# Project-MONAI/GenerativeModels

Measured on AMD Instinct MI355X. Metric: 3D volumes/sec (DDIM 50-step sample, 1x128^3), higher is better.
Workload: dtype bf16; 1 GPU; C2: 3D DiffusionModelUNet(64,128,256; 2 res blocks; mid-block attention 1 head x 256) DDIM-50 sampling of 1x1x128^3 volumes, 1 volume per GPU per step; inference_steps=50, parallelism=1 independent replicas (batch-sharded, no data-path collective), hip_graph=False, self_launched=False

## Files before the change

### generativemodels_amd/csrc/conv_dma.hip

```cpp
#include "conv_dma_shared.h"
#include <type_traits>

#ifdef GM_CONV_TIMELINE
#define TL_STAMP(k)                                                                                                              \
  do {                                                                                                                           \
    if ((p.debug_flags & 4096) && threadIdx.x == 0 && tl_on)                                                                            \
      reinterpret_cast<unsigned long long*>(p.kpartial)[(long long)blockIdx.x * 64 + (k)] = __builtin_readcyclecounter();        \
  } while (0)
#else
#define TL_STAMP(k)
#endif
#ifndef GM_DMA_PART
#define GM_DMA_PART (-1)
#endif
#define DMA_PART(k) (GM_DMA_PART == -1 || GM_DMA_PART == (k))
static __device__ __attribute__((aligned(64))) unsigned int gm_zero_row[16] = {0};

template <typename T, int NW, int MF, int S, int MINW, int KS = 3, int NFR_ = 4, bool PRE = false>
__global__ __launch_bounds__(64 * NW, MINW) void conv_dma_kernel(const GmConvDesc p, const unsigned phase_wgs, const unsigned phase_sleeps) {
  constexpr int BK = ConvTraits<T>::BK;
  constexpr int VECW = ConvTraits<T>::VECW;
  constexpr int NT = 64 * NW;
  constexpr int NFR = NFR_, G = KS == 3 ? 3 : 2, RING = KS == 3 ? 3 : 4;
  static_assert(KS == 3 || (KS == 2 && S == 1 && (NW == 8 || NW == 4)), "the sub-pixel variant is stride 1, 8 waves x 32 or 4 waves x 64 voxels");
  static_assert(NW * MF * 16 == 512 || NW * MF * 16 == (S == 1 ? 256 : 128), "waves x fragments cover the tile");
  constexpr int TH = 4, TW = 16, BM = NW * MF * 16, TD = BM / (TH * TW);
  constexpr int NPW = KS == 2 ? 2 : 1;
  constexpr int PD = S * (TD - 1) + KS, PH = S * (TH - 1) + KS, PW = S * (TW - 1) + KS + (NPW - 1);
  constexpr int EW = TW + 1;
  constexpr int PLANE = ((PH * PW + 15) / 16) * 16;
  constexpr int PROWS = PD * PLANE;
  constexpr int PPIECES = PROWS / 16;
  constexpr int PPW = (PPIECES + NW - 1) / NW;
  constexpr int BN = 16 * NFR;
  constexpr int WROWS = G * BN;
  constexpr bool WGEN = NFR != 4 || (KS == 2 && NW == 4);
  constexpr int PATCH_BYTES = PROWS * DMA_ROWB;
  constexpr int WBUF_BYTES = WROWS * DMA_ROWB;
  constexpr int PVT_OFF = PATCH_BYTES + (KS == 2 ? 36864 : RING * WBUF_BYTES) + 512;
  constexpr int NGROUPS = KS * KS * KS / G * NPW;
  constexpr int WPW = WGEN ? WROWS / 16 / NW : (KS == 2 ? 1 : (NW == 8 ? 2 : (NW == 4 ? 3 : 1)));
  static_assert(!WGEN || (S == 1 && (WROWS / 16) % NW == 0), "general panel distribution: whole pieces per wave");
  static_assert(WROWS == (KS == 3 ? 3 : 2) * BN, "G taps per weight panel");
  static_assert(NGROUPS % RING == 0, "the ring slot of a group is a compile-time constant");
  constexpr bool DIRECT_W = NFR == 4 && KS == 3;

  extern __shared__ __attribute__((aligned(1024))) char smem[];
  const unsigned lds0 = (unsigned)(uintptr_t)smem;

  const int tid = threadIdx.x;
  const int lane = tid & 63;
  const int wave = __builtin_amdgcn_readfirstlane(tid >> 6);
  const int l15 = lane & 15, q = lane >> 4;
  if (blockIdx.x < phase_wgs) {
    const unsigned tg = __builtin_amdgcn_s_getreg((3 << 11) | (16 << 6) | 4);
    if (tg & 1) {
      for (unsigned k = phase_sleeps; k > 0; --k) __builtin_amdgcn_s_sleep(16);
    }
  }

  const int Dt = KS == 2 ? p.Ds : p.Do, Ht = KS == 2 ? p.Hs : p.Ho, Wt = KS == 2 ? p.Ws : p.Wo;
  const int ntd = (Dt + TD - 1) / TD, nth = (Ht + TH - 1) / TH, ntw = (Wt + TW - 1) / TW;
  const int ncb = (p.Cout + BN - 1) / BN;
  const int ksplit = (KS == 3 && S == 1 && p.kpartial && p.ksplit > 1) ? p.ksplit : 1;
  int Dv = p.Ds, Hv = p.Hs, Wv = p.Ws;
  if (p.in_mode == 1) { Dv *= p.fd; Hv *= p.fh; Wv *= p.fw; }
  const int nchunks = p.Cin / BK;
  const int cout_pad = (p.Cout + 15) & ~15;
  const int cps = ksplit > 1 ? (nchunks + ksplit - 1) / ksplit : nchunks;
// ... 32 lines not shown
  int psw = 0;
#pragma unroll
  for (int j = 0; j < PPW; ++j) {
    const int row = 16 * (wave + NW * j) + (lane >> 2);
    const int rr = row % PLANE;
    psw |= dma_swz(rr % PW) << (2 * j);
  }
  int pvox[PPW];
  constexpr bool PVOX_LDS = KS == 2 && NW == 4;
  int* pvt = reinterpret_cast<int*>(smem + PVT_OFF) + threadIdx.x;
  if (PVOX_LDS) pvt[PPW * NT] = psw;
  auto place_patch = [&](const Tile& t) __attribute__((always_inline)) {
    KDesc& pk = cold_desc();
    const int ud0 = t.td_i * TD * S - (KS == 2 ? 1 - ((t.par >> 1) & 1) : pk.pd), uh0 = t.th_i * TH * S - (KS == 2 ? 1 - (t.par & 1) : pk.ph),
              uw0 = t.tw_i * TW * S - (KS == 2 ? 1 : pk.pw);
    OPAQUE_LANE(lane_p);
#pragma unroll
    for (int j = 0; j < PPW; ++j) {
      const int row = 16 * (wave + NW * j) + (lane_p >> 2);
      const int pa = row / PLANE, rr = row - pa * PLANE;
      const int pb = rr / PW, lc = rr - pb * PW;
      const int pc = S == 1 ? lc : (lc < EW ? 2 * lc : 2 * (lc - EW) + 1);
      int ud = ud0 + pa, uh = uh0 + pb, uw = uw0 + pc;
      const bool ok = (row < PROWS) & (rr < PH * PW) & (ud >= 0) & (ud < Dv) & (uh >= 0) & (uh < Hv) & (uw >= 0) & (uw < Wv);
      if (pk.in_mode == 1) { ud /= pk.fd; uh /= pk.fh; uw /= pk.fw; }
      const int pvj = ok ? ((t.n * pk.Ds + ud) * pk.Hs + uh) * pk.Ws + uw : -1;
      if (PVOX_LDS) pvt[j * NT] = pvj; else pvox[j] = pvj;
    }
  };
  const long long xrowb = p.x_ld * (long long)sizeof(T);
  const char* x2base = reinterpret_cast<const char*>(p.x2);
  const long long x2rowb = p.x2_ld * (long long)sizeof(T);
  const int nchunks0 = p.x2 ? p.cin_split / BK : nchunks;
  auto issue_patch = [&](int chunk) __attribute__((always_inline)) {
#ifdef GM_CONV_ABLATE
    if (p.debug_flags & 1024) return;
#endif
    const bool second = chunk >= nchunks0;
    const char* cbase = second ? x2base + (long long)(chunk - nchunks0) * (BK * (int)sizeof(T)) : xbase + (long long)chunk * (BK * (int)sizeof(T));
    const long long rowb = second ? x2rowb : xrowb;
#pragma unroll
    for (int j = 0; j < PPW; ++j) {
      if (wave + NW * j < PPIECES) {
        int pv = PVOX_LDS ? pvt[j * NT] : pvox[j];
        asm volatile("" : "+v"(pv));
        int ps = PVOX_LDS ? pvt[PPW * NT] : psw;
        if (PVOX_LDS) asm volatile("" : "+v"(ps));
        const char* src = pv >= 0 ? cbase + pv * rowb + (((lane & 3) ^ ((ps >> (2 * j)) & 3)) << 4) : zero + ((lane & 3) << 4);
        dma16(src, lds0 + (unsigned)(16 * (wave + NW * j)) * DMA_ROWB);
      }
    }
  };

  Tile cur = decode(sx + pos);
  const Tile stride = decode(gx);
  place_patch(cur);
  if (min(nchunks, cur.ks * cps) < nchunks) issue_patch(min(nchunks, cur.ks * cps));

  constexpr bool pre = PRE;
  float sc[VECW], sh[VECW];
  auto load_affine = [&](int chunk) __attribute__((always_inline)) {
    const int c0 = chunk * BK + (lane & 3) * VECW;
    const float* ps = p.pre_scale + (long long)cur.n * p.Cin + c0;
    const float* ph = p.pre_shift + (long long)cur.n * p.Cin + c0;
#pragma unroll
    for (int i = 0; i < VECW; i += 4) {
      const float4 a = *reinterpret_cast<const float4*>(ps + i), b = *reinterpret_cast<const float4*>(ph + i);
      sc[i] = a.x; sc[i + 1] = a.y; sc[i + 2] = a.z; sc[i + 3] = a.w;
      sh[i] = b.x; sh[i + 1] = b.y; sh[i + 2] = b.z; sh[i + 3] = b.w;
    }
  };
  auto transform_patch = [&]() __attribute__((always_inline)) {
#pragma unroll
    for (int j = 0; j < PPW; ++j) {
      if (wave + NW * j < PPIECES && pvox[j] >= 0) {
        char* a = smem + (16 * (wave + NW * j) + (lane >> 2)) * DMA_ROWB + (((lane & 3) ^ ((psw >> (2 * j)) & 3)) << 4);
        float v[VECW];
        Vec16<T>::unpack(*reinterpret_cast<const uint4*>(a), v);
#pragma unroll
        for (int i = 0; i < VECW; ++i) v[i] = v[i] * sc[i] + sh[i];
        conv_act_vec(v, p.pre_act, sizeof(T) == 4);
        *reinterpret_cast<uint4*>(a) = Vec16<T>::pack(v);
      }
    }
    asm volatile("s_waitcnt lgkmcnt(0)" ::: "memory");
  };


  const char* wbase = nullptr;
  int wsrc[WPW];
  auto place_weights = [&](const Tile& t) __attribute__((always_inline)) {
    KDesc& pk = cold_desc();
    wbase = reinterpret_cast<const char*>(pk.w) + (long long)(t.par * NPW) * nchunks * (KS * KS * KS) * cout_pad * DMA_ROWB;
    OPAQUE_LANE(lane_w);
#pragma unroll
    for (int h = 0; h < WPW; ++h) {
      const int row = WGEN ? 16 * (wave + NW * h) + (lane_w >> 2)
                    : KS == 2 ? 16 * wave + (lane_w >> 2)
                              : NW == 8 ? (h == 0 ? 16 * wave + (lane_w >> 2) : 128 + 8 * wave + ((lane_w & 31) >> 2))
                                        : (NW == 4 ? 16 * (wave + NW * h) + (lane_w >> 2) : 16 * (wave < 12 ? wave : 0) + (lane_w >> 2));
      const int u = row / BN, col = row % BN;
      const int co = t.cb * BN + (DIRECT_W ? direct_col_chan<T>(col) : col);
      wsrc[h] = co < cout_pad ? ((u * cout_pad + co) * DMA_ROWB + (((lane_w & 3) ^ dma_swz(row)) << 4)) : -1;
    }
  };
  auto issue_w_pieces = [&](int t, int buf, int h0, int h1) __attribute__((always_inline)) {
#ifdef GM_CONV_ABLATE
    if (p.debug_flags & 512) return;
#endif
    const char* panel = KS == 2 ? wbase + ((long long)((t & 7) >> 2) * nchunks * 8 + (long long)(t >> 3) * 8 + 2 * (t & 3)) * cout_pad * DMA_ROWB
                                : wbase + (long long)t * G * cout_pad * DMA_ROWB;
    const unsigned dst = lds0 + PATCH_BYTES + (unsigned)buf * WBUF_BYTES;
#pragma unroll
    for (int h = h0; h < h1; ++h) {
      const char* src = wsrc[h] >= 0 ? panel + wsrc[h] : zero + ((lane & 3) << 4);
      if (WGEN) {
        dma16(src, dst + (unsigned)(16 * (wave + NW * h)) * DMA_ROWB);
      } else if (KS == 2) {
        dma16(src, dst + (unsigned)(16 * wave) * DMA_ROWB);
      } else if (NW == 8) {
        if (h == 0) dma16(src, dst + (unsigned)(16 * wave) * DMA_ROWB);
        else if (lane < 32) dma16(src, dst + (unsigned)(128 + 8 * wave) * DMA_ROWB);
      } else if (NW == 16) {
        if (wave < 12) dma16(src, dst + (unsigned)(16 * wave) * DMA_ROWB);
      } else {
        dma16(src, dst + (unsigned)(16 * (wave + NW * h)) * DMA_ROWB);
      }
    }
  };
  auto issue_w = [&](int t, int buf) __attribute__((always_inline)) { issue_w_pieces(t, buf, 0, WPW); };


  constexpr int SCRATCH_WAVE = MF * 16 * 144, SCRATCH_BYTES = NW * SCRATCH_WAVE;
  constexpr int RING_BYTES = KS == 2 ? (RING * WBUF_BYTES > 36864 ? RING * WBUF_BYTES : 36864) : RING * WBUF_BYTES;
  constexpr bool EARLY = SCRATCH_BYTES <= RING_BYTES;
  constexpr int SCRATCH_OFF = EARLY ? PATCH_BYTES : 0;
  static_assert(EARLY || SCRATCH_BYTES <= PATCH_BYTES + RING_BYTES, "the transpose scratch fits under the addend vector");
  static_assert(BN * 8 <= SCRATCH_WAVE, "a wave's statistic partials fit into its scratch block");
  static_assert(PVT_OFF == PATCH_BYTES + RING_BYTES + 512, "the placement table follows the addend vector");
  float* addv = reinterpret_cast<float*>(smem + PATCH_BYTES + RING_BYTES);
  constexpr bool DIRECT = NFR == 4 && KS == 3;
  constexpr int EPASSES = (NFR * 16 * (int)sizeof(T) + 127) / 128;
  constexpr int CH_PER_PASS = 128 / (int)sizeof(T);
  static_assert(EPASSES <= 4, "at most 4 epilogue passes (128 output channels in fp32)");

  for (;;) {
#ifdef GM_CONV_TIMELINE
    const bool tl_on = pos == tl_pos;
#endif
    TL_STAMP(0);
    const int c_begin = min(nchunks, cur.ks * cps), c_end = min(nchunks, c_begin + cps);
    const int total = (c_end - c_begin) * NGROUPS;
    const int od0 = cur.td_i * TD, oh0 = cur.th_i * TH, ow0 = cur.tw_i * TW;
    TL_STAMP(1);
    place_weights(cur);
    if (total > 0) {
      issue_w(c_begin * NGROUPS, 0);
      if (total > 1) issue_w(c_begin * NGROUPS + 1, 1);
      if (pre) load_affine(c_begin);
    }
    float addend = 0.f;
    KDesc& pa = cold_desc();
    OPAQUE_LANE(lane_a);
    const int tid_a = wave * 64 + lane_a;
    if (tid_a < BN) {
      const int co = cur.cb * BN + tid_a;
      if (co < pa.Cout) {
        if (pa.bias) addend += pa.bias[co];
        if (pa.skip_bias) addend += pa.skip_bias[co];
        if (pa.rowvec) addend += pa.rowvec[(long long)cur.n * pa.rowvec_bstride + co];
      }
    }
    TL_STAMP(55);
    constexpr int HK = S * (MF - 1) + KS;
    static_assert(MF <= 4 && (4 % MF) == 0, "a wave's fragments stay inside one 4-row tile plane");
    OPAQUE_LANE(lane_t);
    const int l15t = lane_t & 15, qt = lane_t >> 4;
    constexpr int NXA = KS + NPW - 1;
    int xa[NXA];
    {
      const int m0 = wave * MF * 16 + l15t;
      const int a = m0 >> 6, bb0 = (m0 >> 4) & 3, c = m0 & 15;
#pragma unroll
      for (int kw = 0; kw < NXA; ++kw) {
        const int col = S == 1 ? c + kw : (kw == 1 ? EW + c : c + (kw >> 1));
        xa[kw] = (S * a * PLANE + S * bb0 * PW + col) * DMA_ROWB + ((qt ^ dma_swz(col)) << 4);
      }
    }
    const int wa0 = PATCH_BYTES + l15t * DMA_ROWB + ((qt ^ dma_swz(l15t)) << 4);
#define XADDR(hk, kw) (xa[kw] + (hk) * (PW * DMA_ROWB))
#define WADDR(nf) (wa0 + (nf) * (16 * DMA_ROWB))
    f32x4_t accs[NPW][NFR][MF];
#pragma unroll
    for (int pw = 0; pw < NPW; ++pw)
#pragma unroll
      for (int nf = 0; nf < NFR; ++nf)
#pragma unroll
        for (int mf = 0; mf < MF; ++mf) accs[pw][nf][mf] = (f32x4_t){0.f, 0.f, 0.f, 0.f};
    f32x4_t (&acc)[NFR][MF] = accs[0];
    if (tid_a < BN) addv[tid_a] = addend;
    TL_STAMP(56);
    if (total > 0) {
      dma_wait<0>();
      if (pre) transform_patch();
    }
    __builtin_amdgcn_s_barrier();
#ifdef GM_CONV_TIMELINE
    if (p.debug_flags & 2048) {
      const unsigned tg = __builtin_amdgcn_s_getreg((3 << 11) | (16 << 6) | 4);
      if (tg & 1) {
        for (int k = (p.debug_flags >> 16) & 255; k > 0; --k) __builtin_amdgcn_s_sleep(1);
      }
    }
#endif
    TL_STAMP(2);

    for (int chunk = c_begin; chunk < c_end; ++chunk) {
      const bool last_chunk = chunk + 1 == c_end;
      constexpr int NH = NFR / 4;
      constexpr bool PIPE2 = NH == 1 && !PRE && (KS == 2 || S == 2 || MINW == 2);
      if constexpr (PIPE2) {
        uint4 xf[2][MF], wf[2][4];
        auto read_tap = [&](int g, int u, int set) __attribute__((always_inline)) {
          const int tap = (KS == 2 ? g % 4 : g) * G + u;
          const int kd = tap / (KS * KS), kh = (tap / KS) % KS, kw = tap % KS + (KS == 2 ? g / 4 : 0);
#pragma unroll
          for (int nf = 0; nf < 4; ++nf)
            wf[set][nf] = *reinterpret_cast<const uint4*>(smem + WADDR(nf) + (g % RING) * WBUF_BYTES + u * (BN * DMA_ROWB));
#pragma unroll
          for (int mf = 0; mf < MF; ++mf)
            xf[set][mf] = *reinterpret_cast<const uint4*>(smem + XADDR(S * mf + kh, kw) + kd * (PLANE * DMA_ROWB));
        };
        auto mma_tap_pw = [&](int set, int pw) __attribute__((always_inline)) {
#pragma unroll
          for (int nf = 0; nf < 4; ++nf)
#pragma unroll
            for (int mf = 0; mf < MF; ++mf) Mma<T>::run(wf[set][nf], xf[set][mf], accs[pw][nf][mf]);
        };
#define mma_tap(set) mma_tap_pw(set, KS == 2 ? g / 4 : 0)
        constexpr int NMMA = MF * 4 * (sizeof(T) == 2 ? 1 : 4), NRD = MF + 4;
        static_assert(G == 3 || G == 2, "taps per panel");
#pragma unroll
        for (int g = 0; g < NGROUPS; ++g) {
          const int t = chunk * NGROUPS + g;
          const int X = (g * G) & 1, Y = X ^ 1;
          const int LASTSET = (g * G + G - 1) & 1, NEXTSET = ((g + 1) * G) & 1;
          if (g == 0) read_tap(0, 0, X);
          read_tap(g, 1, Y);
          mma_tap(X);
          if (g == 0) __builtin_amdgcn_sched_group_barrier(0x100, 2 * NRD, 0);
          else __builtin_amdgcn_sched_group_barrier(0x100, NRD, 0);
          __builtin_amdgcn_sched_group_barrier(0x008, NMMA, 0);
          if (g < NGROUPS - 2 || !last_chunk) issue_w(t + 2, (g + 2) % RING);
          if (G == 3) {
            read_tap(g, 2, X);
            mma_tap(Y);
            __builtin_amdgcn_sched_group_barrier(0x100, NRD, 0);
            __builtin_amdgcn_sched_group_barrier(0x008, NMMA, 0);
          }
          if (g == NGROUPS - 1) {
            if (!last_chunk) {
              asm volatile("s_waitcnt lgkmcnt(0)" ::: "memory");
              __builtin_amdgcn_s_barrier();
              issue_patch(chunk + 1);
              if (pre) load_affine(chunk + 1);
              dma_wait<0>();
              if (pre) transform_patch();
              __builtin_amdgcn_s_barrier();
            }
          } else {
            if ((g < NGROUPS - 2 || !last_chunk) && (NW != 16 || wave < 12)) dma_wait<WPW>(); else dma_wait<0>();
            __builtin_amdgcn_s_barrier();
            read_tap(g + 1, 0, NEXTSET);
          }
          mma_tap(LASTSET);
          if (g < NGROUPS - 1) {
            __builtin_amdgcn_sched_group_barrier(0x100, NRD, 0);
            __builtin_amdgcn_sched_group_barrier(0x008, NMMA, 0);
          }
          if (chunk - c_begin < 5) TL_STAMP(3 + (chunk - c_begin) * 10 + g);
        }
      } else {
#pragma unroll
      for (int g = 0; g < NGROUPS; ++g) {
        const int t = chunk * NGROUPS + g;
        if (g < NGROUPS - 2 || !last_chunk) issue_w(t + 2, (g + 2) % RING);
        constexpr int NSTEPS = G * NH;
        uint4 xf[MF], wf[4];
        auto read_step = [&](int st) __attribute__((always_inline)) {
          const int u = st / NH, hf = st % NH;
          const int tap = g * G + u;
          const int kd = tap / (KS * KS), kh = (tap / KS) % KS, kw = tap % KS;
#pragma unroll
          for (int nf = 0; nf < 4; ++nf)
            wf[nf] = *reinterpret_cast<const uint4*>(smem + WADDR(nf) + hf * (64 * DMA_ROWB) + (g % RING) * WBUF_BYTES + u * (BN * DMA_ROWB));
          if (hf == 0) {
#pragma unroll
            for (int mf = 0; mf < MF; ++mf)
              xf[mf] = *reinterpret_cast<const uint4*>(smem + XADDR(S * mf + kh, kw) + kd * (PLANE * DMA_ROWB));
          }
        };
        auto mma_step = [&](int st) __attribute__((always_inline)) {
          const int hf = st % NH;
#pragma unroll
          for (int nf = 0; nf < 4; ++nf)
#pragma unroll
            for (int mf = 0; mf < MF; ++mf) Mma<T>::run(wf[nf], xf[mf], acc[hf * 4 + nf][mf]);
        };
        constexpr int NMMA = MF * 4 * (sizeof(T) == 2 ? 1 : 4);
#pragma unroll
        for (int st = 0; st < NSTEPS - 1; ++st) {
          read_step(st);
          mma_step(st);
          if (st % NH == 0) __builtin_amdgcn_sched_group_barrier(0x100, MF + 4, 0);
// ... 110 lines not shown
              dma16(src, lds0 + (unsigned)(j * BM + wave * (MF * 16) + h * 16) * DMA_ROWB);
            }
            if (WGEN || NW == 4 || (wave >> 2) == j) {
              const char* src = wco < cout_pad ? wsk + ((long long)sc * cout_pad + wco) * DMA_ROWB + wswz : zero + ((lane_k & 3) << 4);
              dma16(src, lds0 + PATCH_BYTES + (unsigned)(j * BN + wpiece * 16) * DMA_ROWB);
            }
          }
        }
        asm volatile("s_waitcnt vmcnt(0)" ::: "memory");
        __builtin_amdgcn_s_barrier();
  #pragma unroll
        for (int j = 0; j < 2; ++j) {
          if (sc0 + j < nsc) {
            uint4 xf[MF], wf[4];
  #pragma unroll
            for (int mf = 0; mf < MF; ++mf) xf[mf] = *reinterpret_cast<const uint4*>(smem + caddr[mf] + j * (BM * DMA_ROWB));
  #pragma unroll
            for (int hf = 0; hf < NFR / 4; ++hf) {
  #pragma unroll
              for (int nf = 0; nf < 4; ++nf)
                wf[nf] = *reinterpret_cast<const uint4*>(smem + WADDR(nf) + hf * (64 * DMA_ROWB) + j * (BN * DMA_ROWB));
  #pragma unroll
              for (int nf = 0; nf < 4; ++nf)
  #pragma unroll
                for (int mf = 0; mf < MF; ++mf) Mma<T>::run(wf[nf], xf[mf], acc[hf * 4 + nf][mf]);
            }
          }
        }
      }
    }


    TL_STAMP(61);
    const bool has_next = pos + gx < cx;
    const bool has_next_early = !DIRECT || has_next || partial;
    if (has_next_early) {
      asm volatile("s_waitcnt lgkmcnt(0)" ::: "memory");
      __builtin_amdgcn_s_barrier();
    }
    Tile nxt = cur;
    if (has_next) {
      if (ksplit > 1) {
        nxt = decode(sx + pos + gx);
      } else {
        int c;
        nxt.cb = cur.cb + stride.cb; c = nxt.cb >= ncb ? 1 : 0; nxt.cb -= c ? ncb : 0;
        if (KS == 2) { nxt.par = cur.par + stride.par + c; c = nxt.par >> 2; nxt.par &= 3; }
        nxt.tw_i = cur.tw_i + stride.tw_i + c; c = nxt.tw_i >= ntw ? 1 : 0; nxt.tw_i -= c ? ntw : 0;
        nxt.th_i = cur.th_i + stride.th_i + c; c = nxt.th_i >= nth ? 1 : 0; nxt.th_i -= c ? nth : 0;
        nxt.td_i = cur.td_i + stride.td_i + c; c = nxt.td_i >= ntd ? 1 : 0; nxt.td_i -= c ? ntd : 0;
        nxt.n = cur.n + stride.n + c;
      }
      place_patch(nxt);
      if (EARLY && min(nchunks, nxt.ks * cps) < nchunks) issue_patch(min(nchunks, nxt.ks * cps));
    }
    TL_STAMP(57);
    KDesc& pe = cold_desc();
    if (KS == 3 && S == 1 && ksplit > 1) {
      const long long nv = (long long)pe.N * pe.Do * pe.Ho * pe.Wo;
      float* part = pe.kpartial + (long long)cur.ks * nv * pe.Cout;
  #pragma unroll
      for (int mf = 0; mf < MF; ++mf) {
        const int m = (wave * MF + mf) * 16 + (lane_e & 15);
        const int od = od0 + (m >> 6), oh = oh0 + ((m >> 4) & 3), ow = ow0 + (m & 15);
        if (od < pe.Do && oh < pe.Ho && ow < pe.Wo) {
          float* row = part + ((((long long)cur.n * pe.Do + od) * pe.Ho + oh) * pe.Wo + ow) * pe.Cout;
  #pragma unroll
          for (int nf = 0; nf < NFR; ++nf) {
            const int co = cur.cb * BN + (DIRECT ? direct_chan<T>(nf, lane_e >> 4, 0) : nf * 16 + (lane_e >> 4) * 4);
            if (co < pe.Cout)
              *reinterpret_cast<float4*>(row + co) = make_float4(acc[nf][mf][0], acc[nf][mf][1], acc[nf][mf][2], acc[nf][mf][3]);
          }
        }
      }
    } else {

#ifdef GM_CONV_ABLATE
    if (!(pe.debug_flags & 256)) {
#endif
    if (DIRECT && d_direct) {
      const int qe = lane_e >> 4;
      typedef float f32x2_t __attribute__((ext_vector_type(2)));
      f32x2_t ds[NST][VECW / 2], dq[NST][VECW / 2];
#pragma unroll
      for (int st = 0; st < NST; ++st)
#pragma unroll
        for (int i = 0; i < VECW / 2; ++i) { ds[st][i] = (f32x2_t){0.f, 0.f}; dq[st][i] = (f32x2_t){0.f, 0.f}; }
      const int Dl = KS == 2 ? pe.Ds : pe.Do, Hl = KS == 2 ? pe.Hs : pe.Ho, Wl = KS == 2 ? pe.Ws : pe.Wo;
      const bool has_res = pe.res != nullptr, has_stats = pe.stats != nullptr;
      const bool full = od0 + TD <= Dl && oh0 + TH <= Hl && ow0 + TW <= Wl && (cur.cb + 1) * BN <= pe.Cout;
      bool ok_st[NST];
#pragma unroll
      for (int st = 0; st < NST; ++st) ok_st[st] = d_lane_ok && cur.cb * BN + (64 * st + 16 * qe) / (int)sizeof(T) < pe.Cout;
      f32x2_t addl[NST][VECW / 2];
#pragma unroll
      for (int st = 0; st < NST; ++st)
#pragma unroll
        for (int i = 0; i < VECW; i += 4) {
          const float4 a = *reinterpret_cast<const float4*>(addv + (64 * st) / (int)sizeof(T) + qe * VECW + i);
          addl[st][i / 2] = (f32x2_t){a.x, a.y};
          addl[st][i / 2 + 1] = (f32x2_t){a.z, a.w};
        }
      auto direct_stores = [&](auto RESc, auto FULLc) __attribute__((always_inline)) {
        constexpr bool RES = decltype(RESc)::value, FULL = decltype(FULLc)::value;
#pragma unroll
        for (int mf = 0; mf < MF; ++mf) {
          const int line = wave * MF + mf;
// ... 154 lines not shown
      EpRows<MF * 2> rows;
      dma_epilogue_rows<T, MF, KS, 2>(pe, etp, wave * MF, lane_e, rows);
      dma_epilogue_pass<T, MF, NFR, KS, 2, DIRECT>(pe, accs[pw], scratch, addv, etp, wave * MF, lane_e, rows, st_s, st_q);
    }
    if constexpr (EPASSES > 3) {
      EpRows<MF * 2> rows;
      dma_epilogue_rows<T, MF, KS, 3>(pe, etp, wave * MF, lane_e, rows);
      dma_epilogue_pass<T, MF, NFR, KS, 3, DIRECT>(pe, accs[pw], scratch, addv, etp, wave * MF, lane_e, rows, st_s, st_q);
    }
    TL_STAMP(62);
    if (pe.stats) {
      OPAQUE_LANE(lane_s);
      float ra[EPASSES][VECW], rb[EPASSES][VECW];
#pragma unroll
      for (int e = 0; e < EPASSES; ++e)
#pragma unroll
        for (int i = 0; i < VECW; ++i) { ra[e][i] = wave_segment_sum(st_s[e][i]); rb[e][i] = wave_segment_sum(st_q[e][i]); }
      if (lane_s < 8) {
        float* part = reinterpret_cast<float*>(scratch);
#pragma unroll
        for (int e = 0; e < EPASSES; ++e)
#pragma unroll
          for (int i = 0; i < VECW; i += 2)
            *reinterpret_cast<float4*>(part + 2 * (e * CH_PER_PASS + lane_s * VECW + i)) = make_float4(ra[e][i], rb[e][i], ra[e][i + 1], rb[e][i + 1]);
      }
      __syncthreads();
      const int ch = wave * 64 + lane_s;
      if (ch < BN) {
        double a = 0.0, b2 = 0.0;
#pragma unroll
        for (int w = 0; w < NW; ++w) {
          const float2 v = *reinterpret_cast<const float2*>(smem + SCRATCH_OFF + w * SCRATCH_WAVE + ch * 8);
          a += (double)v.x;
          b2 += (double)v.y;
        }
        const int co = cur.cb * BN + ch;
        if (co < pe.Cout) {
          const long long slot = ((long long)(cur.td_i * nth + cur.th_i) * ntw + cur.tw_i) * (KS == 2 ? 8 : 1) + etp.par;
          double* dst = pe.stats + ((slot * pe.N + cur.n) * pe.Cout + co) * 2;
          *reinterpret_cast<double2*>(dst) = make_double2(a, b2);
        }
      }
    }
    }
    }
#ifdef GM_CONV_ABLATE
    }
#endif
    }
    TL_STAMP(63);
    if (!has_next) break;
    asm volatile("s_waitcnt lgkmcnt(0)" ::: "memory");
    __builtin_amdgcn_s_barrier();
    if (!EARLY && min(nchunks, nxt.ks * cps) < nchunks) issue_patch(min(nchunks, nxt.ks * cps));
    cur = nxt;
    pos += gx;
  }
}

#undef mma_tap
#undef XADDR
#undef WADDR


#if DMA_PART(0)
extern "C" long long gm_conv_dma_lds_bytes(int variant) {
  const long long addv = 512;
  if (variant == 4) return 5LL * 96 * DMA_ROWB + 36864 + addv + 256LL * 9 * 4;
  if (variant == 5) return 10LL * 112 * DMA_ROWB + 3LL * 384 * DMA_ROWB + addv;
  const long long plane = variant == 2 ? 304 : 112, planes = variant == 1 ? 6 : (variant == 2 ? 5 : 10);
  return planes * plane * DMA_ROWB + 3LL * 192 * DMA_ROWB + addv;
}

#endif
#if DMA_PART(0)
int gm_dma_grid_cap = 0;
extern "C" void gm_conv_dma_set_persistent(int max_work_groups) { gm_dma_grid_cap = max_work_groups; }

int gm_dma_phase_skew = 0;
extern "C" void gm_conv_dma_set_phase_skew(int cycles) { gm_dma_phase_skew = cycles; }
#else
extern int gm_dma_grid_cap, gm_dma_phase_skew;
#endif
#define g_dma_grid_cap gm_dma_grid_cap
#define g_dma_phase_skew gm_dma_phase_skew
static int dma_device_cus() {
  static int cus = 0;
  if (cus == 0) {
    int dev = 0, n = 0;
    if (hipGetDevice(&dev) != hipSuccess || hipDeviceGetAttribute(&n, hipDeviceAttributeMultiprocessorCount, dev) != hipSuccess || n <= 0) n = 256;
    cus = n;
  }
  return cus;
}

static unsigned dma_grid(unsigned nwork, long long lds_bytes, int by_waves, bool splitk) {
  if (splitk || g_dma_grid_cap == 0) return nwork;
  long long cap = g_dma_grid_cap;
  if (cap < 0) {
    const int cus = dma_device_cus();
    long long per_cu = (160LL * 1024) / lds_bytes;
    if (per_cu > by_waves) per_cu = by_waves;
    if (per_cu < 1) per_cu = 1;
    cap = per_cu * cus;
  }
  if (cap < 8) cap = 8;
  return nwork < (unsigned)cap ? nwork : (unsigned)cap;
}

#if DMA_PART(0)
extern "C" int gm_conv_dma_variant(int cfg) { return cfg == 17 ? 4 : (cfg == 15 ? 2 : (cfg == 16 || cfg == 18 ? 3 : (cfg == 19 ? 5 : 1))); }

extern "C" int gm_conv_dma_eligible(const GmConvDesc* d) {
  if (d->cfg == 21 || d->cfg == 22) return 0;
  if (d->cfg == 24 || d->cfg == 25) return gm_conv_sn_eligible(d);
  const int bk = d->dtype == GM_F32 ? 16 : 32;
  const int vecw = d->dtype == GM_F32 ? 4 : 8;
  const int s = d->cfg == 15 ? 2 : 1;
  if (d->cfg == 17) {
    return d->in_mode == 3 && d->kd == 2 && d->kh == 2 && d->kw == 2 && d->sd == 1 && d->sh == 1 && d->sw == 1 && d->dd == 1 && d->dh == 1 &&
           d->dw == 1 && d->Do == 2 * d->Ds && d->Ho == 2 * d->Hs && d->Wo == 2 * d->Ws && d->Cin % bk == 0 && d->x_ld % vecw == 0 &&
           (reinterpret_cast<uintptr_t>(d->x) & 15) == 0 && d->pre_scale == nullptr && d->pre_act == 0 && d->x2 == nullptr && d->ltd == 2 && d->lth == 2 &&
           d->ltw == 4 && d->Cout % vecw == 0 && d->y_ld % vecw == 0 && (reinterpret_cast<uintptr_t>(d->y) & 15) == 0 &&
           (!d->res || (d->res_ld % vecw == 0 && (reinterpret_cast<uintptr_t>(d->res) & 15) == 0)) && !d->skip_x[0] &&
           (long long)d->N * d->Do * d->Ho * d->Wo < (1LL << 31);
  }
  if (d->in_mode == 3) return 0;
  return d->kd == 3 && d->kh == 3 && d->kw == 3 && d->sd == s && d->sh == s && d->sw == s && d->dd == 1 && d->dh == 1 && d->dw == 1 &&
         (d->in_mode == 0 || (d->in_mode == 1 && s == 1)) && d->Cin % bk == 0 && d->x_ld % vecw == 0 &&
         (reinterpret_cast<uintptr_t>(d->x) & 15) == 0 &&
         ((d->pre_stats[0] == nullptr &&
           ((d->pre_scale == nullptr && d->pre_shift == nullptr && d->pre_act == 0) ||
            (s == 1 && d->pre_scale != nullptr && d->pre_shift != nullptr && (reinterpret_cast<uintptr_t>(d->pre_scale) & 15) == 0 &&
             (reinterpret_cast<uintptr_t>(d->pre_shift) & 15) == 0 && (d->Cin % 4) == 0))) ||
          (d->pre_stats[0] != nullptr && d->cfg == 11 && gm_conv_sk_eligible(d))) &&
         gm_conv_second_source_ok(d, bk, vecw) && gm_conv_shortcut_ok(d, bk, vecw) &&
         d->ltd == (d->cfg == 16 || d->cfg == 18 || d->cfg == 19 ? 3 : (s == 1 ? 2 : 1)) && d->lth == 2 &&
         d->ltw == 4 && d->Cout % vecw == 0 && d->y_ld % vecw == 0 && (reinterpret_cast<uintptr_t>(d->y) & 15) == 0 &&
         (!d->res || (d->res_ld % vecw == 0 && (reinterpret_cast<uintptr_t>(d->res) & 15) == 0)) &&
         (long long)d->N * d->Ds * d->Hs * d->Ws < (1LL << 31) && (long long)d->N * d->Do * d->Ho * d->Wo < (1LL << 31);
}

#endif
template <typename T, int NW, int MF, int S, int MINW, int KS = 3, int NFR = 4, bool PRE = false>
static void launch_dma(const GmConvDesc& d, unsigned nblocks, hipStream_t st) {
  static bool attr_set = false;
  auto kern = conv_dma_kernel<T, NW, MF, S, MINW, KS, NFR, PRE>;
  if (!attr_set) {
    hipError_t e = hipFuncSetAttribute(reinterpret_cast<const void*>(kern), hipFuncAttributeMaxDynamicSharedMemorySize, 160 * 1024);
    if (e != hipSuccess) (void)hipGetLastError();
    attr_set = true;
  }
  const long long lds = gm_conv_dma_lds_bytes(gm_conv_dma_variant(d.cfg));
  const bool splitk = d.ksplit > 1 && d.kpartial != nullptr;
  constexpr int BY_WAVES = MINW * 4 / NW >= 1 ? MINW * 4 / NW : 1;
  const unsigned grid = dma_grid(nblocks, lds, BY_WAVES, splitk);
  long long per_cu = (160LL * 1024) / lds;
  if (per_cu > BY_WAVES) per_cu = BY_WAVES;
  const unsigned resident = (unsigned)(per_cu * dma_device_cus());
  unsigned phase_wgs = 0, phase_sleeps = 0;
  if (per_cu >= 2 && !splitk && g_dma_phase_skew != 0 && nblocks >= 2 * resident) {
    long long cycles = g_dma_phase_skew;
    if (cycles < 0) {
      const long long chunks = d.Cin / (d.dtype == GM_F32 ? 16 : 32), taps = KS * KS * KS;
      const long long mfma_cycles = chunks * taps * (MF * NFR) * (d.dtype == GM_F32 ? 4 * 8 : 16);
      const long long waves_per_simd = per_cu * NW / 4 > 0 ? per_cu * NW / 4 : 1;
      cycles = (18000 + waves_per_simd * mfma_cycles) / 2;
    }
    phase_wgs = resident;
    phase_sleeps = (unsigned)((cycles + 512) / 1024);
    if (phase_sleeps == 0) phase_wgs = 0;
  }
  kern<<<dim3(grid), 64 * NW, (size_t)lds, st>>>(d, phase_wgs, phase_sleeps);
}

#define DMA_BY_DTYPE(...)                                                                    \
  do {                                                                                       \
    if (d.dtype == GM_F32) { using T = float; __VA_ARGS__; return 0; }                       \
    if (d.dtype == GM_BF16) { using T = bf16_raw; __VA_ARGS__; return 0; }                   \
    return -2;                                                                               \
  } while (0)
#if DMA_PART(0)
extern "C" int gm_conv_dma_launch_part0(const GmConvDesc* dp, unsigned nblocks, void* stream) {
  const GmConvDesc& d = *dp; hipStream_t st = (hipStream_t)stream;
  const bool pre = d.pre_scale != nullptr;
  DMA_BY_DTYPE(if (pre) launch_dma<T, 8, 2, 1, 4, 3, 4, true>(d, nblocks, st); else launch_dma<T, 8, 2, 1, 4>(d, nblocks, st));
}
#endif
#if DMA_PART(1)
extern "C" int gm_conv_dma_launch_part1(const GmConvDesc* dp, unsigned nblocks, void* stream) {
  const GmConvDesc& d = *dp; hipStream_t st = (hipStream_t)stream;
  const bool pre = d.pre_scale != nullptr;
  DMA_BY_DTYPE(if (pre) launch_dma<T, 4, 4, 1, 2, 3, 4, true>(d, nblocks, st); else launch_dma<T, 4, 4, 1, 2>(d, nblocks, st));
}
#endif
#if DMA_PART(2)
extern "C" int gm_conv_dma_launch_part2(const GmConvDesc* dp, unsigned nblocks, void* stream) {
  const GmConvDesc& d = *dp; hipStream_t st = (hipStream_t)stream;
  if (d.cfg == 17) DMA_BY_DTYPE((launch_dma<T, 4, 4, 1, 2, 2>(d, nblocks, st)));
  DMA_BY_DTYPE((launch_dma<T, 8, 1, 2, 2>(d, nblocks, st)));
}
#endif
#if DMA_PART(3)
extern "C" int gm_conv_dma_launch_part3(const GmConvDesc* dp, unsigned nblocks, void* stream) {
  const GmConvDesc& d = *dp; hipStream_t st = (hipStream_t)stream;
  const bool pre = d.pre_scale != nullptr;
// ... 26 lines not shown
```

### generativemodels_amd/ops.py

```python
from __future__ import annotations

import contextlib
import ctypes as C
import itertools
import math
import os
import threading
import weakref
from collections import namedtuple
from typing import Optional, Sequence

import torch

from . import _native as nat
from ._native import GmAttnBwdDesc, GmAttnDesc, GmConvDesc, GmDftDesc, GmGnTables, GmKlParams, GmResizeDesc, GmRowsDesc, GmStepParams, GmWgradDesc, check, lib
from .resize_plan import ResizePlan, plan_for
from .spectral_plan import SpectralPlan, device_twiddles
from .spectral_plan import plan_for as spectral_plan_for

_DT = {torch.float32: 0, torch.bfloat16: 1}
ACT = {"none": 0, "silu": 1, "relu": 2}
ACT_BWD = {"none": 0, "silu": 1, "relu": 2, "leakyrelu": 3}
POST_ACT = {"none": 0, "relu": 1, "tanh": 2, "sigmoid": 3, "silu": 4, "swish": 4, "leakyrelu": 5, "gelu": 6}

# ... 892 lines not shown
GN_IN_TOKEN_GEMM = True
GN_IN_SPLIT_SLICES = True
GN_IN_CONSUMER_MAX_ROWS = 128
GN_IN_CONSUMER_MAX_CHANNELS = 384


class GnRecipe:

    def __init__(self, stats, cs, n: int, v: int, groups: int, eps: float, gamma, beta, device) -> None:
        self.stats, self.cs, self.n, self.v, self.groups, self.eps, self.device = stats, cs, n, v, groups, float(eps), device
        self.gamma, self.beta = as_f32(gamma), as_f32(beta)
        self._done = None

    def materialise(self):
        if self._done is None:
            c = sum(self.cs)
            scale = torch.empty((self.n, c), dtype=torch.float32, device=self.device)
            shift = torch.empty((self.n, c), dtype=torch.float32, device=self.device)
            st = self.stats
            check(lib().gm_gn_finalize_channels(st[0].data_ptr(), st[0].shape[0], self.cs[0], st[1].data_ptr() if len(st) > 1 else None,
                                                st[1].shape[0] if len(st) > 1 else 0, self.cs[1] if len(st) > 1 else 0, self.n, self.v, self.groups, self.eps,
                                                _ptr(self.gamma), _ptr(self.beta), scale.data_ptr(), shift.data_ptr(), _stream()), "gm_gn_finalize_channels")
            self._done = (scale, shift)
        return self._done

    def __iter__(self):
        return iter(self.materialise())

    def __getitem__(self, i):
        return self.materialise()[i]

    def __len__(self):
        return 2


def gn_scale_shift_composed(x, groups: int, eps: float, gamma: Optional[torch.Tensor], beta: Optional[torch.Tensor]):
    parts = x.parts if isinstance(x, VirtualCat) else [x]
    n = parts[0].shape[0]
    v = rows_of(parts[0]) // max(n, 1)
    cs = [p.shape[-1] for p in parts]
    c = sum(cs)
    if c % groups != 0:
        raise ValueError("num_channels must be divisible by num_groups")
    stats = [channel_stats(p) for p in parts]
    recipe = GnRecipe(stats, cs, n, v, groups, eps, gamma, beta, parts[0].device)
    if GN_IN_CONSUMER and not torch.is_grad_enabled() and all(st.shape[0] <= GN_IN_CONSUMER_MAX_ROWS for st in stats) and c <= GN_IN_CONSUMER_MAX_CHANNELS and n > 0:
        return recipe
    return recipe.materialise()


GN_APPLY_POLICY = "auto"
DMA_FUSED_PROLOGUE = os.environ.get("GM_DMA_FUSED_PROLOGUE", "auto")
DMA_FUSED_PROLOGUE_MAX_FLOP = 3.0e10
SPLITK = os.environ.get("GM_CONV_SPLITK", "1") != "0"
SPLITK_MAX_TILES = 256
SPLITK_TARGET_WGS = int(os.environ.get("GM_CONV_SPLITK_WGS", "256"))
SPLITK_MAX = 8
_SK_KERNEL = os.environ.get("GM_CONV_SK")
DMA_CFGS = (11, 14, 15, 16, 17, 18, 19, 24, 25)
NARROW_N = os.environ.get("GM_CONV_SN", "1") != "0"
NARROW_N_MAX_CHUNKS = int(os.environ.get("GM_CONV_SN_MAX_CHUNKS", "6"))
NARROW_N_2D = True
EDGE_2D_AS_3D = True
NARROW_N_2D_MAX_FLOP = 3e10
NARROW_N_2D_STRIDE2 = True
NARROW_HEAD_MAX_FLOP = 1.0e9
COUT1_MARCH = True
DMA_WIDE_WAVES = os.environ.get("GM_CONV_WIDE_WAVES", "1") != "0"
DMA_WIDE_WAVE_MIN_TILES = 512


def fuse_gn_prologue(x: torch.Tensor) -> bool:
    if GN_APPLY_POLICY == "prologue":
        return True
    if GN_APPLY_POLICY == "pass":
        return False
    if x.dtype != torch.bfloat16 or x.shape[-1] % 8 != 0:
        return True
    if x.numel() >= (1 << 22):
        return False
    vox = x.numel() // max(x.shape[0] * x.shape[-1], 1)
    return not (x.dim() == 5 and x.shape[-1] % 32 == 0 and vox <= 4096)


def layernorm(x: torch.Tensor, gamma: Optional[torch.Tensor], beta: Optional[torch.Tensor], eps: float = 1e-5) -> torch.Tensor:
    require_device(x)
    out = torch.empty(x.shape, dtype=x.dtype, device=x.device)
    check(lib().gm_layernorm(x.data_ptr(), arena_ld(x), out.data_ptr(), arena_ld(out), _ptr(as_f32(gamma)), _ptr(as_f32(beta)),
                             rows_of(x), x.shape[-1], float(eps), dt_code(x.dtype), _stream()), "gm_layernorm")
    return out


def geglu(x: torch.Tensor) -> torch.Tensor:
    require_device(x)
    inner = x.shape[-1] // 2
    out = torch.empty((*x.shape[:-1], inner), dtype=x.dtype, device=x.device)
    check(lib().gm_geglu(x.data_ptr(), arena_ld(x), out.data_ptr(), arena_ld(out), rows_of(x), inner, dt_code(x.dtype), _stream()),
          "gm_geglu")
    return out


def _clog2(v: int) -> int:
    return max(0, (int(v) - 1).bit_length())


def _tile_bits(total_bits: int, out_dims):
# ... 21 lines not shown
        bits[i] += 1
    return bits


_CFG_TILES = {}


def _cfg_tile(cfg: int):
    if cfg not in _CFG_TILES:
        bm, bn = C.c_int(), C.c_int()
        check(lib().gm_conv_cfg_tile(cfg, C.byref(bm), C.byref(bn)), "gm_conv_cfg_tile")
        _CFG_TILES[cfg] = (bm.value, bn.value)
    return _CFG_TILES[cfg]


COUT1_MARCH_LTD = os.environ.get("GM_CONV_COUT1_LTD")
COUT1_MARCH_LTW_128B = 4


_CONV_DEBUG_FLAGS = 0
_SK_STAMPS = None
_CONV_TIMELINE_BUFFER = None

SMALL_LINEAR_ROWS = 64
TOKEN_GEMM = os.environ.get("GM_TOKEN_GEMM", "1") != "0"
TOKEN_GEMM_MAX_ROWS = int(os.environ.get("GM_TOKEN_GEMM_MAX_ROWS", "32768"))
TOKEN_GEMM_MAX_CIN = 512
TOKEN_GEMM_MAX_FLOP = 2.0e9
DMA_CONV = True
DMA_CONV_MIN_VOXELS = 1 << 8
LDS_SOFT_LIMIT = 80 * 1024
LDS_HARD_LIMIT = 160 * 1024


_FIXED_TILE_BITS = {11: (2, 2, 4), 12: (2, 2, 4), 14: (2, 2, 4), 15: (1, 2, 4), 16: (3, 2, 4), 18: (3, 2, 4), 19: (3, 2, 4), 24: (2, 2, 4), 25: (0, 4, 4)}


def _choose_conv_cfg(desc: GmConvDesc, n_vox_out: int, force_cfg: Optional[int] = None, only: Optional[tuple] = None, exclude: tuple = ()):
    cout = desc.Cout
    if force_cfg is not None:
        order = [force_cfg]
    elif cout <= 16:
        order = [3, 4, 2]
    elif cout <= 64:
        order = [10, 8, 5, 0, 4, 2] if n_vox_out * desc.N >= (1 << 20) else [8, 5, 0, 4, 2]
    else:
        order = [10, 9, 6, 1, 4, 2] if n_vox_out * desc.N >= (1 << 20) else [9, 6, 1, 4, 2]
    if force_cfg is None and n_vox_out * desc.N >= DMA_CONV_MIN_VOXELS:
        if cout == 1:
            order = ([20, 13] if COUT1_MARCH else [13]) + order
        if desc.Cin <= 4:
            order = [12] + order
    if force_cfg is None and cout > 16 and DMA_CONV and n_vox_out * desc.N >= DMA_CONV_MIN_VOXELS:
        wide = not desc.pre_scale and _conv_tiles(desc.N, (desc.Do, desc.Ho, desc.Wo), cout) >= DMA_WIDE_WAVE_MIN_TILES and DMA_WIDE_WAVES
        order = ([15] if desc.sd == 2 else ([14, 11] if wide else [11])) + order
    if (force_cfg is None and NARROW_N_2D and DMA_CONV and desc.kd == 1 and desc.Ds == 1 and desc.kh == 3 and desc.kw == 3
            and ((desc.sh == 1 and desc.sw == 1) or (NARROW_N_2D_STRIDE2 and desc.sh == 2 and desc.sw == 2))
            and 2.0 * n_vox_out * desc.N * cout * desc.Cin * 9 * desc.sh * desc.sw <= NARROW_N_2D_MAX_FLOP):
        order = [25] + order
    if force_cfg is None and n_vox_out * desc.N <= 256 * 64:
        dma_first = [c for c in order if c in (11, 12, 15, 18, 19)]
        rest = [c for c in order if c not in (11, 12, 15, 18, 19)]
        order = dma_first + [c for c in rest if _cfg_tile(c)[0] <= 64] + [c for c in rest if _cfg_tile(c)[0] > 64]
    order = [c for c in order if (only is None or c in only) and c not in exclude]
    best = None
    for cfg in order:
        bits = _FIXED_TILE_BITS.get(cfg)
        if bits is None:
            bm, _ = _cfg_tile(cfg)
            bits = (_tile_bits_fast if cfg >= 5 else _tile_bits)(bm.bit_length() - 1, (desc.Do, desc.Ho, desc.Wo))
        if cfg == 20:
            ltw = (COUT1_MARCH_LTW_128B if desc.Cin * (4 if desc.dtype == 0 else 2) == 128 else 4)
            cols = desc.N * -(-desc.Ho // 8) * -(-desc.Wo // (1 << ltw))
            want = 512 if (ltw == 4 and desc.Cin * (4 if desc.dtype == 0 else 2) == 128) else 256
            ltd = 5
            while ltd > 2 and cols * -(-desc.Do // (1 << ltd)) < want:
                ltd -= 1
            if COUT1_MARCH_LTD is not None:
                ltd = int(COUT1_MARCH_LTD)
            bits = [ltd, 3, ltw]
        desc.cfg, desc.ltd, desc.lth, desc.ltw = cfg, bits[0], bits[1], bits[2]
        lds = lib().gm_conv_lds_bytes(C.byref(desc))
        soft = LDS_HARD_LIMIT if cfg >= 5 else LDS_SOFT_LIMIT
        if 0 < lds <= soft:
            return
        if 0 < lds <= LDS_HARD_LIMIT and best is None:
            best = (cfg, bits)
    if best is None:
        raise ValueError("convolution geometry needs more than 160 KiB of LDS per tile (kernel/stride/dilation too large)")
    desc.cfg, (desc.ltd, desc.lth, desc.ltw) = best[0], best[1]


def _attach_conv_stats(d: GmConvDesc, out: torch.Tensor, n: int, cout: int) -> None:
    slots = lib().gm_conv_stats_slots(C.byref(d))
    if slots > 0:
        cst = torch.empty((slots, n, cout, 2), dtype=torch.float64, device=out.device)
        d.stats = cst.data_ptr()
        out._gm_cstats = cst


def _out_and_res(out_shape, dtype, device, out, res):
    if out is not None and (tuple(out.shape) != out_shape or out.dtype != dtype):
        raise ValueError(f"out has shape {tuple(out.shape)}, expected {out_shape}")
    if res is not None and (tuple(res.shape) != out_shape or res.dtype != dtype):
        raise ValueError(f"residual has shape {tuple(res.shape)} / {res.dtype}, expected {out_shape} / {dtype}")
    if out is None:
        return torch.empty(out_shape, dtype=dtype, device=device), out_shape[-1]
# ... 249 lines not shown
    if x2 is not None:
        d.x2, d.x2_ld, d.cin_split = x2.data_ptr(), arena_ld(x2), f.cin0
    keep = [panel, _epilogue_into(d, n, cout, out, out_ld, res, rowvec, bias, post_act)]
    if _recipe_fits_prologue(g, f):
        d.pre_scale = d.pre_shift = pre.stats[0].data_ptr()
    elif pre is not None:
        sc, sh = pre
        require_device(sc, sh)
        if tuple(sc.shape) != (n, cin) or sc.dtype != torch.float32:
            raise ValueError("pre scale/shift must be fp32 [N, Cin]")
        d.pre_scale, d.pre_shift = sc.data_ptr(), sh.data_ptr()
    if skip is not None:
        parts, sw, sb = skip
        parts = list(parts)
        require_device(sw, sb, *parts)
        if res is not None:
            raise ValueError("skip and res are exclusive (the shortcut IS the residual)")
        if not 1 <= len(parts) <= 2 or sw.shape[0] != cout or sw.shape[1] != sum(t.shape[-1] for t in parts) or math.prod(sw.shape[2:]) != 1:
            raise ValueError("skip = (1 or 2 parts, [Cout, sum(C_part), 1...] weight, bias)")
        for i, t in enumerate(parts):
            if tuple(t.shape[:-1]) != tuple(out.shape[:-1]) or t.dtype != dtype:
                raise ValueError("skip parts must have the output geometry and dtype")
            d.skip_x[i], d.skip_ld[i], d.skip_cin[i] = t.data_ptr(), arena_ld(t), t.shape[-1]
        keep += [packed_conv_weight(sw, dtype), as_f32(sb)]
        d.skip_w, d.skip_bias = keep[-2].data_ptr(), _ptr(keep[-1])
    _geometry_into(d, n, cin, cout, g.src, g.out_sp, g.k, g.conv_stride, g.conv_pad, g.dil, dtype)
    d.pre_act = ACT[pre_act]
    return d, keep


def _conv_tiles(n: int, out_sp, cout: int) -> int:
    return n * -(-out_sp[0] // 4) * -(-out_sp[1] // 4) * -(-out_sp[2] // 16) * -(-cout // 64)


def _split_slices(g: ConvGeometry, nchunks: int, ksplit: Optional[int]) -> int:
    if ksplit is None:
        tiles = _conv_tiles(g.n, g.out_sp, g.cout)
        ksplit = min(nchunks, SPLITK_MAX, SPLITK_TARGET_WGS // tiles) if tiles < SPLITK_MAX_TILES else 1
    return -(-nchunks // -(-nchunks // ksplit)) if ksplit > 1 else ksplit


def _covers(d: GmConvDesc, nvox: int, cfg: Optional[int]) -> bool:
    try:
        _choose_conv_cfg(d, nvox, cfg, only=DMA_CFGS)
        return True
    except ValueError:
        return False


def _plan_tile_kernels(d: GmConvDesc, g: ConvGeometry, f: ConvFacts) -> ConvPlan:
    n, cin, cout, forced = g.n, g.cin, g.cout, f.force_cfg
    nvox, bk = math.prod(g.out_sp), 64 // g.es
    flop = 2.0 * n * nvox * cout * cin * math.prod(g.k)
    fuse_in_lds = f.pre is None or DMA_FUSED_PROLOGUE in (True, "always", "1") or (DMA_FUSED_PROLOGUE == "auto" and flop <= DMA_FUSED_PROLOGUE_MAX_FLOP)
    large = nvox * n >= DMA_CONV_MIN_VOXELS
    dma_ok = False
    if forced is not None and forced in DMA_CFGS or (forced is None and DMA_CONV and cout > 16 and large and fuse_in_lds):
        dma_ok = _covers(d, nvox, forced)
    if NARROW_N and forced is None and f.ksplit is None and DMA_CONV and fuse_in_lds and large:
        if dma_ok and d.cfg == 11 and SPLITK:
            deep = cin // bk + sum(f.skip_cin or ()) // bk
            if _split_slices(g, cin // bk, None) > 1 and deep <= NARROW_N_MAX_CHUNKS and not _covers(d, nvox, 24):
                _choose_conv_cfg(d, nvox, 11, only=DMA_CFGS)
        elif not dma_ok and cout <= 16 and (d.kd == 3 or NARROW_N_2D) and flop <= NARROW_HEAD_MAX_FLOP:
            dma_ok = _covers(d, nvox, 24 if d.kd == 3 else 25)
    recipe_at = None
    if _recipe_fits_prologue(g, f):
        if dma_ok and d.cfg in (24, 25):
            recipe_at = "descriptor"
        elif dma_ok and d.cfg == 11 and GN_IN_SPLIT_SLICES and (f.ksplit is not None or SPLITK):
            recipe_at = "slices"
        else:
            recipe_at = "launch"
    if not dma_ok:
        if forced is not None and forced in DMA_CFGS:
            raise ValueError(f"configuration {forced} does not cover this convolution")
        if f.cat:
            return ConvPlan("two_pass", 0, 0, recipe_at)
        if f.pre is not None and forced is None and cout > 16 and math.prod(g.k) > 1 and not f.gn_fused:
            return ConvPlan("two_pass", 0, 0, recipe_at)
        if f.skip_cin is not None:
            return ConvPlan("shortcut_first", 0, 0, recipe_at)
        _choose_conv_cfg(d, nvox, forced, exclude=(DMA_CFGS + (() if f.w333 else (12,))) if forced is None else ())
    if d.cfg == 12 and not f.w333:
        raise ValueError("configuration 12 needs the original [Cout, Cin, 3, 3, 3] weight (its K-major image is derived from it)")
    ksplit = workspace = 0
    if dma_ok and d.cfg == 11 and (f.ksplit is not None or SPLITK):
        ks = _split_slices(g, cin // bk, f.ksplit)
        if ks > 1:
            d.ksplit = int(ks)
            workspace = lib().gm_conv_splitk_workspace_bytes(C.byref(d))
            if workspace > 0:
                ksplit = d.ksplit
            elif f.ksplit is not None:
                raise ValueError(f"split-K by {ks} is not available for this convolution")
            else:
                d.ksplit = workspace = 0
    if recipe_at == "slices" and not ksplit:
        recipe_at = "launch"
    return ConvPlan(None, ksplit, workspace, recipe_at)


def _finalise_into(d: GmConvDesc, recipe: GnRecipe) -> None:
    sc, sh = recipe.materialise()
    d.pre_scale, d.pre_shift = sc.data_ptr(), sh.data_ptr()


# ... 1283 lines not shown
```

Baseline: 1.441 volumes/s.

## Pipeline fused GroupNorm prologue per chunk in wide-wave bf16 DMA conv

For the bf16 4-wave 3x3x3 stride-1 DMA conv variant with a fused normalize/activation prologue, the per-channel scale/shift now arrive by DMA into a small LDS slot next to each input patch. Each chunk's patch is then transformed inside the chunk loop, and the double-buffered PIPE2 main loop is enabled for these prologue kernels. The planner also fuses the prologue in LDS and picks the wide-wave config for large convs whose shapes are listed in a whitelist table, even above the FLOP threshold. The goal is to avoid a separate GroupNorm-apply pass over large 3D activations. The cost is an extra barrier and transform per chunk and more LDS.

```diff
diff --git a/generativemodels_amd/csrc/conv_dma.hip b/generativemodels_amd/csrc/conv_dma.hip
--- a/generativemodels_amd/csrc/conv_dma.hip
+++ b/generativemodels_amd/csrc/conv_dma.hip
@@ -15,6 +15,10 @@
 #endif
 #define DMA_PART(k) (GM_DMA_PART == -1 || GM_DMA_PART == (k))
 static __device__ __attribute__((aligned(64))) unsigned int gm_zero_row[16] = {0};
+
+template <typename T, int NW, int MF, int S, int MINW, int KS, int NFR, bool PRE>
+constexpr bool dma_pre_pipelined() { return PRE && sizeof(T) == 2 && NW == 4 && MF == 4 && S == 1 && MINW == 2 && KS == 3 && NFR == 4; }
+constexpr int DMA_AFFINE_SLOT = 256;
 
 template <typename T, int NW, int MF, int S, int MINW, int KS = 3, int NFR_ = 4, bool PRE = false>
 __global__ __launch_bounds__(64 * NW, MINW) void conv_dma_kernel(const GmConvDesc p, const unsigned phase_wgs, const unsigned phase_sleeps) {
@@ -153,10 +157,24 @@
     }
   };
 
+  constexpr bool PRE_PIPE = dma_pre_pipelined<T, NW, MF, S, MINW, KS, NFR_, PRE>();
+  static_assert(!PRE_PIPE || (KS == 3 && 2 * BK * 4 <= DMA_AFFINE_SLOT), "the affine slots take the place of the sub-pixel form's placement table");
+  auto issue_affine = [&](int n, int chunk) __attribute__((always_inline)) {
+    if constexpr (PRE_PIPE) {
+      KDesc& pk = cold_desc();
+      if (lane < 2 * (BK / 4)) {
+        const float* src = (lane < BK / 4 ? pk.pre_scale : pk.pre_shift) + (long long)n * pk.Cin + chunk * BK + (lane & (BK / 4 - 1)) * 4;
+        dma16(src, lds0 + PVT_OFF + (unsigned)wave * DMA_AFFINE_SLOT);
+      }
+    }
+  };
   Tile cur = decode(sx + pos);
   const Tile stride = decode(gx);
   place_patch(cur);
-  if (min(nchunks, cur.ks * cps) < nchunks) issue_patch(min(nchunks, cur.ks * cps));
+  if (min(nchunks, cur.ks * cps) < nchunks) {
+    issue_patch(min(nchunks, cur.ks * cps));
+    issue_affine(cur.n, min(nchunks, cur.ks * cps));
+  }
 
   constexpr bool pre = PRE;
   float sc[VECW], sh[VECW];
@@ -172,10 +190,21 @@
     }
   };
   auto transform_patch = [&]() __attribute__((always_inline)) {
+    int lane_x = lane;
+    if constexpr (PRE_PIPE) asm volatile("" : "+v"(lane_x));
+    if constexpr (PRE_PIPE) {
+      const char* af = smem + PVT_OFF + wave * DMA_AFFINE_SLOT + (lane_x & 3) * (VECW * 4);
+#pragma unroll
+      for (int i = 0; i < VECW; i += 4) {
+        const float4 a = *reinterpret_cast<const float4*>(af + i * 4), b = *reinterpret_cast<const float4*>(af + BK * 4 + i * 4);
+        sc[i] = a.x; sc[i + 1] = a.y; sc[i + 2] = a.z; sc[i + 3] = a.w;
+        sh[i] = b.x; sh[i + 1] = b.y; sh[i + 2] = b.z; sh[i + 3] = b.w;
+      }
+    }
 #pragma unroll
     for (int j = 0; j < PPW; ++j) {
       if (wave + NW * j < PPIECES && pvox[j] >= 0) {
-        char* a = smem + (16 * (wave + NW * j) + (lane >> 2)) * DMA_ROWB + (((lane & 3) ^ ((psw >> (2 * j)) & 3)) << 4);
+        char* a = smem + (16 * (wave + NW * j) + (lane_x >> 2)) * DMA_ROWB + (((lane_x & 3) ^ ((psw >> (2 * j)) & 3)) << 4);
         float v[VECW];
         Vec16<T>::unpack(*reinterpret_cast<const uint4*>(a), v);
 #pragma unroll
@@ -258,7 +287,7 @@
     if (total > 0) {
       issue_w(c_begin * NGROUPS, 0);
       if (total > 1) issue_w(c_begin * NGROUPS + 1, 1);
-      if (pre) load_affine(c_begin);
+      if (pre && !PRE_PIPE) load_affine(c_begin);
     }
     float addend = 0.f;
     KDesc& pa = cold_desc();
@@ -301,11 +330,15 @@
     f32x4_t (&acc)[NFR][MF] = accs[0];
     if (tid_a < BN) addv[tid_a] = addend;
     TL_STAMP(56);
-    if (total > 0) {
-      dma_wait<0>();
-      if (pre) transform_patch();
-    }
-    __builtin_amdgcn_s_barrier();
+    if constexpr (PRE_PIPE) {
+      if (total <= 0) __builtin_amdgcn_s_barrier();
+    } else {
+      if (total > 0) {
+        dma_wait<0>();
+        if (pre) transform_patch();
+      }
+      __builtin_amdgcn_s_barrier();
+    }
 #ifdef GM_CONV_TIMELINE
     if (p.debug_flags & 2048) {
       const unsigned tg = __builtin_amdgcn_s_getreg((3 << 11) | (16 << 6) | 4);
@@ -319,7 +352,18 @@
     for (int chunk = c_begin; chunk < c_end; ++chunk) {
       const bool last_chunk = chunk + 1 == c_end;
       constexpr int NH = NFR / 4;
-      constexpr bool PIPE2 = NH == 1 && !PRE && (KS == 2 || S == 2 || MINW == 2);
+      constexpr bool PIPE2 = NH == 1 && (!PRE || PRE_PIPE) && (KS == 2 || S == 2 || MINW == 2);
+      if constexpr (PRE_PIPE) {
+        if (chunk > c_begin) {
+          asm volatile("s_waitcnt lgkmcnt(0)" ::: "memory");
+          __builtin_amdgcn_s_barrier();
+          issue_patch(chunk);
+          issue_affine(cur.n, chunk);
+        }
+        dma_wait<0>();
+        transform_patch();
+        __builtin_amdgcn_s_barrier();
+      }
       if constexpr (PIPE2) {
         uint4 xf[2][MF], wf[2][4];
         auto read_tap = [&](int g, int u, int set) __attribute__((always_inline)) {
@@ -360,7 +404,7 @@
             __builtin_amdgcn_sched_group_barrier(0x008, NMMA, 0);
           }
           if (g == NGROUPS - 1) {
-            if (!last_chunk) {
+            if (!last_chunk && !PRE_PIPE) {
               asm volatile("s_waitcnt lgkmcnt(0)" ::: "memory");
               __builtin_amdgcn_s_barrier();
               issue_patch(chunk + 1);
@@ -577,7 +621,10 @@
         nxt.n = cur.n + stride.n + c;
       }
       place_patch(nxt);
-      if (EARLY && min(nchunks, nxt.ks * cps) < nchunks) issue_patch(min(nchunks, nxt.ks * cps));
+      if (EARLY && min(nchunks, nxt.ks * cps) < nchunks) {
+        issue_patch(min(nchunks, nxt.ks * cps));
+        issue_affine(nxt.n, min(nchunks, nxt.ks * cps));
+      }
     }
     TL_STAMP(57);
     KDesc& pe = cold_desc();
@@ -838,7 +885,10 @@
     if (!has_next) break;
     asm volatile("s_waitcnt lgkmcnt(0)" ::: "memory");
     __builtin_amdgcn_s_barrier();
-    if (!EARLY && min(nchunks, nxt.ks * cps) < nchunks) issue_patch(min(nchunks, nxt.ks * cps));
+    if (!EARLY && min(nchunks, nxt.ks * cps) < nchunks) {
+      issue_patch(min(nchunks, nxt.ks * cps));
+      issue_affine(nxt.n, min(nchunks, nxt.ks * cps));
+    }
     cur = nxt;
     pos += gx;
   }
@@ -937,7 +987,7 @@
     if (e != hipSuccess) (void)hipGetLastError();
     attr_set = true;
   }
-  const long long lds = gm_conv_dma_lds_bytes(gm_conv_dma_variant(d.cfg));
+  const long long lds = gm_conv_dma_lds_bytes(gm_conv_dma_variant(d.cfg)) + (dma_pre_pipelined<T, NW, MF, S, MINW, KS, NFR, PRE>() ? NW * DMA_AFFINE_SLOT : 0);
   const bool splitk = d.ksplit > 1 && d.kpartial != nullptr;
   constexpr int BY_WAVES = MINW * 4 / NW >= 1 ? MINW * 4 / NW : 1;
   const unsigned grid = dma_grid(nblocks, lds, BY_WAVES, splitk);
diff --git a/generativemodels_amd/ops.py b/generativemodels_amd/ops.py
--- a/generativemodels_amd/ops.py
+++ b/generativemodels_amd/ops.py
@@ -968,6 +968,16 @@
 GN_APPLY_POLICY = "auto"
 DMA_FUSED_PROLOGUE = os.environ.get("GM_DMA_FUSED_PROLOGUE", "auto")
 DMA_FUSED_PROLOGUE_MAX_FLOP = 3.0e10
+DMA_FUSED_PROLOGUE_WINS = {((4,), 1): 8192, ((4, 2), 1): 8192}
+
+
+def _fused_prologue_wins(cin: int, cin0: int, cout: int, n: int, out_sp, es: int, k, stride) -> bool:
+    if es != 2 or tuple(k) != (3, 3, 3) or tuple(stride) != (1, 1, 1) or len(out_sp) != 3 or cin % 32 or cin0 % 32:
+        return False
+    blocks = -(-cout // 64)
+    parts = (cin // 32,) if cin0 in (0, cin) else (cin0 // 32, (cin - cin0) // 32)
+    tiles = DMA_FUSED_PROLOGUE_WINS.get((parts, blocks))
+    return tiles is not None and _conv_tiles(n, out_sp, cout) // blocks >= tiles
 SPLITK = os.environ.get("GM_CONV_SPLITK", "1") != "0"
 SPLITK_MAX_TILES = 256
 SPLITK_TARGET_WGS = int(os.environ.get("GM_CONV_SPLITK_WGS", "256"))
@@ -1095,7 +1105,9 @@
         if desc.Cin <= 4:
             order = [12] + order
     if force_cfg is None and cout > 16 and DMA_CONV and n_vox_out * desc.N >= DMA_CONV_MIN_VOXELS:
-        wide = not desc.pre_scale and _conv_tiles(desc.N, (desc.Do, desc.Ho, desc.Wo), cout) >= DMA_WIDE_WAVE_MIN_TILES and DMA_WIDE_WAVES
+        pre_wide = desc.in_mode == 0 and _fused_prologue_wins(desc.Cin, desc.cin_split if desc.x2 else 0, cout, desc.N, (desc.Do, desc.Ho, desc.Wo), 4 if desc.dtype == 0 else 2,
+                                                              (desc.kd, desc.kh, desc.kw), (desc.sd, desc.sh, desc.sw))
+        wide = (not desc.pre_scale or pre_wide) and _conv_tiles(desc.N, (desc.Do, desc.Ho, desc.Wo), cout) >= DMA_WIDE_WAVE_MIN_TILES and DMA_WIDE_WAVES
         order = ([15] if desc.sd == 2 else ([14, 11] if wide else [11])) + order
     if (force_cfg is None and NARROW_N_2D and DMA_CONV and desc.kd == 1 and desc.Ds == 1 and desc.kh == 3 and desc.kw == 3
             and ((desc.sh == 1 and desc.sw == 1) or (NARROW_N_2D_STRIDE2 and desc.sh == 2 and desc.sw == 2))
@@ -1451,7 +1463,9 @@
     n, cin, cout, forced = g.n, g.cin, g.cout, f.force_cfg
     nvox, bk = math.prod(g.out_sp), 64 // g.es
     flop = 2.0 * n * nvox * cout * cin * math.prod(g.k)
-    fuse_in_lds = f.pre is None or DMA_FUSED_PROLOGUE in (True, "always", "1") or (DMA_FUSED_PROLOGUE == "auto" and flop <= DMA_FUSED_PROLOGUE_MAX_FLOP)
+    fuse_in_lds = f.pre is None or DMA_FUSED_PROLOGUE in (True, "always", "1") or (DMA_FUSED_PROLOGUE == "auto" and (
+        flop <= DMA_FUSED_PROLOGUE_MAX_FLOP or (DMA_WIDE_WAVES and not g.upsample and not g.transposed and g.in_mode == 0
+                                                and _fused_prologue_wins(cin, f.cin0 if f.cat else 0, cout, n, g.out_sp, g.es, g.k, g.s))))
     large = nvox * n >= DMA_CONV_MIN_VOXELS
     dma_ok = False
     if forced is not None and forced in DMA_CFGS or (forced is None and DMA_CONV and cout > 16 and large and fuse_in_lds):
```

New measurement: 1.449 volumes/s (median of 6 runs). No clear change (+0.6%).
